# DEEPDIP-project/IncompressibleNavierStokes.jl

Hardware: AMD Instinct MI355X
Metric: M lattice-cell updates/sec (RK4 step incl. Poisson), 3D TGV fp64 (higher is better)
Workload: dtype f64; 1 GPU; TaylorGreenVortex3D 256^3 periodic fp64, RK44 + spectral Poisson, dt=0.001, Re=1e3; decomposition=single GPU, loop=timesteps_ (K steps, one native call)

## Files before the change

include/ins_hip.h:

```cpp
#ifndef INS_HIP_H
#define INS_HIP_H

#include <stdint.h>

#ifdef __cplusplus
extern "C" {
#endif

#define INS_OK 0
#define INS_ERR_INVALID (-1)
#define INS_ERR_HIP (-2)
#define INS_ERR_FFT (-3)
#define INS_ERR_UNSUPPORTED (-4)
#define INS_ERR_NOCONV (-5)
#define INS_ERR_COMM (-6)

#define INS_BC_PERIODIC 0
#define INS_BC_DIRICHLET 1
#define INS_BC_SYMMETRIC 2
#define INS_BC_PRESSURE 3
#define INS_BC_HALO 4

typedef struct ins_grid ins_grid_t;
typedef struct ins_poisson ins_poisson_t;
// ... 77 lines not shown

int ins_rk_create(const ins_grid_t* grid, ins_poisson_t* ps, int nstage, const double* A, const double* c, ins_rk_t** out);
int ins_rk_destroy(ins_rk_t* rk);
int ins_rk_step_f64(ins_rk_t* rk, double visc, double* u, double t, double dt, const double* const* planes, void* stream);
int ins_rk_step_bc_f64(ins_rk_t* rk, double visc, double* u, double t, double dt, const double* const* planes_by_time, void* stream);
int ins_rk_steps_f64(ins_rk_t* rk, double visc, double* u, double t, double dt, int nsteps, void* stream);
int ins_combine_f64(const ins_grid_t* grid, const double* base, double* out, int nterms, const double* coefs,
                    const double* const* ks, void* stream);
int ins_rk_profile_enable(ins_rk_t* rk, int enable);
int ins_rk_profile_read(ins_rk_t* rk, double* momentum_ms, int64_t* momentum_launches);
int ins_rk_set_bodyforce(ins_rk_t* rk, const double* force);

int ins_dbg_stage_rhs_used(const ins_rk_t* rk, int64_t* launches);
int ins_dbg_stage_rhs(ins_rk_t* rk, double visc, const double* u_in, const double* pI, const double* ustart, const double* kterm, double coef_k,
                      double self_in, double coef_self, double* ustar, double* rhs, int32_t* used, void* stream);
int ins_rk_pressure(const ins_rk_t* rk, double** p);
int ins_rk_stage_force(const ins_rk_t* rk, int i, double** ku);

int ins_vorticity_f64(const ins_grid_t* grid, const double* u, double* w, void* stream);
int ins_interpolate_u_p_f64(const ins_grid_t* grid, const double* u, double* up, void* stream);
int ins_interpolate_w_p_f64(const ins_grid_t* grid, const double* w, double* wp, void* stream);
int ins_dfield_f64(const ins_grid_t* grid, const double* p, double* G, double* d, double eps, void* stream);
int ins_qfield_f64(const ins_grid_t* grid, const double* u, double* Q, void* stream);
int ins_dissipation_from_strain_f64(const ins_grid_t* grid, double visc, const double* u, double* eps_out, void* stream);
int ins_eig2field_f64(const ins_grid_t* grid, const double* u, double* lam, void* stream);
int ins_apply_bc_temp_f64(const ins_grid_t* grid, const int32_t* bc, const double* val, const double* const* planes, double* temp, void* stream);
int ins_convection_diffusion_temp_f64(const ins_grid_t* grid, double a4, const double* u, const double* temp, double* c, void* stream);
int ins_dissipation_f64(const ins_grid_t* grid, double visc, double coef, const double* u, double* diff, double* diss, void* stream);
int ins_gravity_f64(const ins_grid_t* grid, int gdir, double a2, const double* temp, double* F, void* stream);
int ins_smagtensor_f64(const ins_grid_t* grid, double theta, const double* u, double* sigma, void* stream);
// ... 132 lines not shown
```

incompressiblenavierstokes.jl_amd/_lib.py:

```python
import ctypes as C
import os

_HERE = os.path.dirname(os.path.abspath(__file__))
LIB_PATH = os.environ.get("INS_HIP_LIB") or os.path.join(_HERE, "libinship.so")

INS_BC_PERIODIC, INS_BC_DIRICHLET, INS_BC_SYMMETRIC, INS_BC_PRESSURE, INS_BC_HALO = range(5)

c_double_p = C.POINTER(C.c_double)
vp = C.c_void_p


class GridDesc(C.Structure):

    _fields_ = [
        ("D", C.c_int32),
        ("N", C.c_int32 * 3),
        ("dx", c_double_p * 3),
        ("dxu", c_double_p * 3),
        ("A1", (c_double_p * 3) * 3),
        ("A2", (c_double_p * 3) * 3),
        ("iu_lo", (C.c_int32 * 3) * 3),
        ("iu_hi", (C.c_int32 * 3) * 3),
        ("ip_lo", C.c_int32 * 3),
        ("ip_hi", C.c_int32 * 3),
# ... 83 lines not shown
    "ins_filter_face_f64": (C.c_int, [vp, vp, C.c_int, vp, vp, vp]),
    "ins_filter_volume_f64": (C.c_int, [vp, vp, C.c_int, vp, vp, vp]),
    "ins_reconstruct_f64": (C.c_int, [vp, vp, C.c_int, vp, vp, vp]),
    "ins_filter_face_pullback_f64": (C.c_int, [vp, vp, C.c_int, vp, vp, vp]),
    "ins_filter_volume_pullback_f64": (C.c_int, [vp, vp, C.c_int, vp, vp, vp]),
    "ins_rk_create": (C.c_int, [vp, vp, C.c_int, c_double_p, c_double_p, C.POINTER(vp)]),
    "ins_rk_destroy": (C.c_int, [vp]),
    "ins_rk_step_f64": (C.c_int, [vp, C.c_double, vp, C.c_double, C.c_double, C.POINTER(vp), vp]),
    "ins_rk_step_bc_f64": (C.c_int, [vp, C.c_double, vp, C.c_double, C.c_double, C.POINTER(vp), vp]),
    "ins_rk_steps_f64": (C.c_int, [vp, C.c_double, vp, C.c_double, C.c_double, C.c_int, vp]),
    "ins_combine_f64": (C.c_int, [vp, vp, vp, C.c_int, c_double_p, C.POINTER(vp), vp]),
    "ins_rk_profile_enable": (C.c_int, [vp, C.c_int]),
    "ins_rk_profile_read": (C.c_int, [vp, c_double_p, C.POINTER(C.c_int64)]),
    "ins_rk_set_bodyforce": (C.c_int, [vp, vp]),
    "ins_dbg_stage_rhs_used": (C.c_int, [vp, C.POINTER(C.c_int64)]),
    "ins_dbg_stage_rhs": (C.c_int, [vp, C.c_double, vp, vp, vp, vp, C.c_double, C.c_double, C.c_double, vp, vp, C.POINTER(C.c_int32), vp]),
    "ins_rk_pressure": (C.c_int, [vp, C.POINTER(vp)]),
    "ins_rk_stage_force": (C.c_int, [vp, C.c_int, C.POINTER(vp)]),
    "ins_rk_set_temperature": (C.c_int, [vp, vp]),
    "ins_rk_set_closure": (C.c_int, [vp, C.c_int32, C.c_double]),
    "ins_rk_step_ext_f64": (C.c_int, [vp, C.c_double, vp, vp, C.c_double, C.c_double, vp]),
    "ins_stage_momentum_f64": (C.c_int, [vp, C.c_double, vp, vp, vp, vp, C.c_int, c_double_p, C.POINTER(vp), C.c_double, vp]),
    "ins_stage_momentum_corr_f64": (C.c_int, [vp, C.c_double, vp, vp, vp, vp, vp, C.c_int, c_double_p, C.POINTER(vp), C.c_double, vp]),
    "ins_stage_momentum_corr_part_f64": (C.c_int, [vp, C.c_double, vp, vp, vp, vp, vp, C.c_int, c_double_p, C.POINTER(vp), C.c_double, C.c_double, C.c_double, vp, C.c_int, vp]),
    "ins_slab_divergence_f64": (C.c_int, [vp, vp, vp, vp]),
    "ins_slab_applypressure_f64": (C.c_int, [vp, vp, vp, vp, vp]),
    "ins_slab_fft_create": (C.c_int, [C.POINTER(C.c_int32), c_double_p, C.c_int, C.c_int, C.POINTER(vp)]),
    "ins_slab_fft_destroy": (C.c_int, [vp]),
    "ins_slab_fft_sizes": (C.c_int, [vp, C.POINTER(C.c_int64), C.POINTER(C.c_int64)]),
    "ins_slab_fft_forward_xy": (C.c_int, [vp, vp, vp, vp, vp]),
# ... 136 lines not shown
```

incompressiblenavierstokes.jl_amd/csrc/ins_flux64.hip:

```cpp
#include <algorithm>
#include <cstdlib>
#include <cstring>

#include "ins_internal.h"
#include "ins_wave64.h"
#include "ins_flux_common.h"

namespace {

template <typename T, int R>
struct Plane {
  T v[3][R + 2];
  T h[3];
  T raw[3][R];
  T vm2;
  T rawv0;
};

template <typename T, int R>
struct TExt {
  T t[R + 2];
  T th;
  T vm1;
};

template <typename T, int R, int XW, bool FUSE, int CORR, bool SKEL = false, int NW = 4, bool EXTRA = false, bool RHS = false>
__global__ __launch_bounds__(64 * NW, NW == 16 ? 4 : 2) void k_flux64(FluxArgs a) {
  static_assert(!RHS || (FUSE && CORR <= 1 && !SKEL && !EXTRA), "right-hand side in the stage kernel: fused epilogue, periodic box, no extra terms");
  constexpr unsigned EB = (unsigned)sizeof(T);
  const T* const a_u = static_cast<const T*>(a.u);
  const T* const a_pI = static_cast<const T*>(a.pI);
  T* const a_F = static_cast<T*>(a.F);
  static_assert(R + 2 + (CORR ? 1 : 0) <= 8, "packed halo rows live in 8-lane groups");
  int txi, tyi, tzi;
  {
    const int nty_local = (a.nty + 7) >> 3;
    int seq = (int)(blockIdx.x >> 3);
    if (seq >= a.ntx * nty_local * a.ntz) return;
    txi = seq % a.ntx;
    seq /= a.ntx;
    tyi = (int)(blockIdx.x & 7) * nty_local + seq % nty_local;
    tzi = seq / nty_local;
    if (tyi >= a.nty) return;
// ... 69 lines not shown
    const rsrc_t rt = plane_rsrc(static_cast<const T*>((const void*)a.te.temp) + po, ubytes);
#pragma unroll
    for (int rr = 0; rr < R + 2; ++rr) E.t[rr] = ldb<T>(rt, ucol, urow[rr]);
    E.th = ldb<T>(rt, uhoff, 0);
    E.vm1 = ldb<T>(plane_rsrc(a_u + po + a.sc, ubytes), ucol, urowm1);
  };
  constexpr int NPR = R + 3 + (RHS ? 1 : 0);
  auto load_p = [&](T (&P)[NPR], T& PH, int kk) {
    const rsrc_t rs = plane_rsrc(a_pI + (long long)(CORR == 2 ? min(kk, N2) : wrapi(kk - 1, n2)) * n0 * n1, qbytes);
#pragma unroll
    for (int rr = 0; rr < R + 3; ++rr) P[rr] = ldb<T>(rs, qcol, qrow[rr]);
    PH = ldb<T>(rs, qhoff, 0);
    if constexpr (RHS) P[R + 3] = ldb<T>(rs, qcol, qrowm2);
  };
  auto correct = [&](Plane<T, R>& P, const T (&Pc)[NPR], T PHc, const T (&Pn)[NPR], T PHn) {
    if (a.epi.self_in != 0.0) {
#pragma unroll
      for (int c = 0; c < 3; ++c)
#pragma unroll
        for (int rr = 0; rr < R; ++rr) P.raw[c][rr] = P.v[c][rr + 1];
      if constexpr (RHS) P.rawv0 = P.v[1][0];
    }
    if constexpr (RHS) P.vm2 -= (Pc[0] - Pc[R + 3]) * Y.gs;
#pragma unroll
    for (int rr = 0; rr < R + 2; ++rr) {
      const T pc = Pc[rr];
      P.v[0][rr] -= (next_h(pc, rdlane(PHc, 16 + rr)) - pc) * X.gs;
      P.v[1][rr] -= (Pc[rr + 1] - pc) * Y.gs;
      P.v[2][rr] -= (Pn[rr] - pc) * Z.gs;
    }
    P.h[0] -= (dpp_old<0x108>(PHc, PHc) - PHc) * X.gs;
// ... 257 lines not shown
              if (xout && j < n1) {
                const long long pk = (long long)k * sz;
                if (a.te.ktemp_out) stb(plane_rsrc(static_cast<T*>((void*)a.te.ktemp_out) + pk, ubytes), ocol, orow[rr - 1], kt);
                stb(plane_rsrc(static_cast<T*>((void*)a.te.temp_out) + pk, ubytes), ocol, orow[rr - 1], tacc[rr - 1] + (T)a.te.c_self * kt);
              }
              wv_o = wv;
              wwprev[rr - 1] = ww;
              Tz[rr - 1] = Tc;
            }
          }
          Pz[0][rr - 1] = Uc;
          Pz[1][rr - 1] = Vc;
          Pz[2][rr - 1] = Wc;
        }
        emit(rr, k, fu, fv, fw, FUSE ? sacc[0][rr - 1] : (T)0, FUSE ? sacc[1][rr - 1] : (T)0, FUSE ? sacc[2][rr - 1] : (T)0, st);
        if constexpr (RHS) {
          const T su = sacc[0][rr - 1] + (T)a.epi.coef_self * fu, sv = sacc[1][rr - 1] + (T)a.epi.coef_self * fv, sw = sacc[2][rr - 1] + (T)a.epi.coef_self * fw;
          us_u[rr - 1] = su;
          dvs[rr - 1] = sv - vs_o;
          dws[rr - 1] = sw - wsprev[rr - 1];
          vs_o = sv;
          wsprev[rr - 1] = sw;
          if (lane == 63) rhs_lds[((k & 1) * NW + wave) * R + rr - 1] = su;
        }
      } else if constexpr (RHS) {
        const T fyv_m = flux(cvm2, Vc, cvm2, Vc, Y.vs);
        const T fxv = flux(Vc, Vn, Uc, C.v[0][rr + 1], X.vo);
        const T lxv = flux(rdlane(ch1, rr), Vc, rdlane(ch0, rr), rdlane(ch0, rr + 1), X.vo);
        T fv = (fxv - prev_h(fxv, lxv)) * X.ro;
        fv += (fyv - fyv_m) * Y.rs;
// ... 165 lines not shown
        INS_LAUNCH_CHECK();
        return INS_OK;
      }
      if (corr_mode == 1) {
        hipLaunchKernelGGL((k_flux64<T, R, XW, true, 1, false, NW, true>), dim3(nb), block, (size_t)g_lds, s, a);
        INS_LAUNCH_CHECK();
        return INS_OK;
      }
    }
    ins_set_error("stage kernel with an extra force term: fp64, fused epilogue, 2 rows, 4 wavefronts, no slab correction");
    return INS_ERR_UNSUPPORTED;
  }
  if (corr_mode == 0)
    hipLaunchKernelGGL((k_flux64<T, R, XW, FUSE, 0, false, NW>), dim3(nb), block, (size_t)g_lds, s, a);
  else if constexpr (FUSE && R <= 5) {
    if (corr_mode == 1)
      hipLaunchKernelGGL((k_flux64<T, R, XW, true, 1, false, NW>), dim3(nb), block, (size_t)g_lds, s, a);
    else
      hipLaunchKernelGGL((k_flux64<T, R, XW, true, 2, false, NW>), dim3(nb), block, (size_t)g_lds, s, a);
  } else {
    ins_set_error("in-kernel pressure correction needs the fused epilogue and <= 5 rows per thread");
    return INS_ERR_UNSUPPORTED;
  }
  INS_LAUNCH_CHECK();
  return INS_OK;
}

constexpr int ZB = 4;
template <typename T, int R, int XW, bool FUSE, int NW = 4>
int launch(const ins_grid* G, FluxArgs& a, int corr_mode, int part, hipStream_t s) {
  const GridDev& g = G->g;
// ... 6 lines not shown
  if (part != 0 && nzl <= 2 * ZB) {
    if (part == 1) return INS_OK;
    part = 0;
  }
  if (part == 1) {
    a.k_lo = 1 + ZB;
    a.k_hi = nzl + 1 - ZB;
  } else if (part == 2) {
    a.zc = ZB;
    a.kB = nzl + 1 - ZB;
  }
  a.ntz = part == 2 ? 2 : cdiv(a.k_hi - a.k_lo, a.zc);
  return launch_range<T, R, XW, FUSE, NW>(G, a, corr_mode, s);
}

template <int R, int XW, int NW, int CORR>
int launch_rhs(const ins_grid* G, FluxArgs& a, hipStream_t s) {
  const GridDev& g = G->g;
  a.ntx = 1;
  a.nty = cdiv(g.N[1] - 2, (NW / XW) * R);
  a.k_lo = 1;
  a.k_hi = g.N[2] - 1;
  a.kB = 0;
  a.ntz = cdiv(a.k_hi - a.k_lo, a.zc);
  const unsigned nb = (unsigned)(8LL * ((a.nty + 7) / 8) * a.ntz);
  hipLaunchKernelGGL((k_flux64<double, R, XW, true, CORR, false, NW, false, true>), dim3(nb), dim3(64, NW, 1), 0, s, a);
  INS_LAUNCH_CHECK();
  return INS_OK;
}

}

extern "C" void ins_tune_flux64(int disable, int rows, int rows_corr, int zchunk, int xw, int skel, int burst_unused, int lds) {
  if (disable >= 0) ins_set_option("INS_DISABLE_FLUX64", disable);
  if (rows >= 0) ins_set_option("INS_FLUX64_ROWS", rows);
  if (rows_corr >= 0) ins_set_option("INS_FLUX64_ROWS_CORR", rows_corr);
  if (zchunk >= 0) ins_set_option("INS_FLUX64_ZC", zchunk);
  if (xw >= 0) ins_set_option("INS_FLUX64_XW", xw);
  if (skel >= 0) ins_set_option("INS_FLUX64_SKEL", skel);
  (void)burst_unused;
  if (lds >= 0) ins_set_option("INS_FLUX64_LDS", lds);
// ... 54 lines not shown
    if (!zco) zc = n2 >= 128 ? 32 : (n2 >= 64 ? 16 : (n2 >= 32 ? 8 : 4));
  }
  return TileShape{xw, rows, nw, zc};
}

bool ins_flux128_supported(const ins_grid* G, const RkEpi* epi, int corr_mode, bool f32);
bool ins_flux64_stage_rhs_supported(const ins_grid* G, int corr_mode) {
  if (ins_opt(OPT_INS_DISABLE_STAGE_RHS) || corr_mode < 0 || corr_mode > 1 || !ins_flux64_supported(G) || g_skel || g_lds) return false;
  if (ins_flux128_supported(G, nullptr, corr_mode, false)) return false;
  const TileShape t = tile_shape(G, corr_mode, false, false, true);
  if (64 * t.xw != G->g.N[0] - 2) return false;
  if (corr_mode == 0) return t.rows == 4 && t.xw == 2 && t.nw == 4;
  return t.rows == 2 && ((t.xw == 3 && t.nw == 6) || ((t.xw == 2 || t.xw == 4) && (t.nw == 4 || t.nw == 8)));
}

template <typename T>
static int flux64_dispatch(const ins_grid* G, double visc, const T* u, T* F, const RkEpi* epi, const T* pI, int corr_mode, hipStream_t s, int part) {
  const GridDev& g = G->g;
  FluxArgs a;
  memset(&a, 0, sizeof(a));
  a.u = u;
  a.pI = pI;
  a.F = F;
  a.sc = g.sc;
  a.N0 = g.N[0];
  a.N1 = g.N[1];
  a.N2 = g.N[2];
  a.X = make_dir(G, 0, visc);
  a.Y = make_dir(G, 1, visc);
  a.Z = make_dir(G, 2, visc);
// ... 22 lines not shown
          if (xw == 4) return launch<T, RR, 4, FUSE, 16>(G, a, corr_mode, part, s);   \
          if (xw == 2) return launch<T, RR, 2, FUSE, 16>(G, a, corr_mode, part, s);   \
          return launch<T, RR, 1, FUSE, 16>(G, a, corr_mode, part, s);                \
        }                                                                             \
      }                                                                               \
      if (nw >= 8) {                                                                  \
        if (xw == 4) return launch<T, RR, 4, FUSE, 8>(G, a, corr_mode, part, s);      \
        if (xw == 2) return launch<T, RR, 2, FUSE, 8>(G, a, corr_mode, part, s);      \
        return launch<T, RR, 1, FUSE, 8>(G, a, corr_mode, part, s);                   \
      }                                                                               \
      if (xw == 4) return launch<T, RR, 4, FUSE>(G, a, corr_mode, part, s);           \
      if (xw == 2) return launch<T, RR, 2, FUSE>(G, a, corr_mode, part, s);           \
      return launch<T, RR, 1, FUSE>(G, a, corr_mode, part, s);                        \
    }                                                                                 \
  }
  if (want_rhs) {
    if (ins_stage_out_aliases_input(*epi, u)) {
      ins_set_error("stage kernel asked for the Poisson right-hand side while u* overwrites one of its inputs");
      return INS_ERR_INVALID;
    }
    if constexpr (!F32) {
      if (part == 0 && ins_flux64_stage_rhs_supported(G, corr_mode)) {
        a.rdiv[0] = 1.0 / G->desc.dx[0][1];
        a.rdiv[1] = 1.0 / G->desc.dx[1][1];
        a.rdiv[2] = 1.0 / G->desc.dx[2][1];
        a.om = G->desc.dx[0][1] * G->desc.dx[1][1] * G->desc.dx[2][1];
        if (corr_mode == 0) return launch_rhs<4, 2, 4, 0>(G, a, s);
        if (xw == 3) return launch_rhs<2, 3, 6, 1>(G, a, s);
        if (xw == 4) return nw == 8 ? launch_rhs<2, 4, 8, 1>(G, a, s) : launch_rhs<2, 4, 4, 1>(G, a, s);
        return nw == 8 ? launch_rhs<2, 2, 8, 1>(G, a, s) : launch_rhs<2, 2, 4, 1>(G, a, s);
      }
    }
    ins_set_error("stage kernel asked for the Poisson right-hand side on a box or tile shape it does not write it for");
    return INS_ERR_UNSUPPORTED;
  }
  if (epi) {
    INS_F64_CASE(2, true)
    INS_F64_CASE(3, true)
    INS_F64_CASE(4, true)
    INS_F64_CASE(5, true)
    INS_F64_CASE(6, true)
  } else {
// ... 1 lines not shown
    INS_F64_CASE(3, false)
    INS_F64_CASE(4, false)
    INS_F64_CASE(5, false)
    INS_F64_CASE(6, false)
  }
#undef INS_F64_CASE
  return INS_ERR_INVALID;
}

bool ins_flux128_supported(const ins_grid* G, const RkEpi* epi, int corr_mode, bool f32);
int ins_k_flux128(const ins_grid* G, double visc, const double* u, double* F, const RkEpi* epi, const double* pI, int corr_mode, hipStream_t s, int part);
int ins_k_flux128_f32(const ins_grid* G, double visc, const float* u, float* F, const RkEpi* epi, const float* pI, int corr_mode, hipStream_t s, int part);

int ins_k_flux64(const ins_grid* G, double visc, const double* u, double* F, const RkEpi* epi, const double* pI, int corr_mode, hipStream_t s,
                 int part) {
  if (ins_flux128_supported(G, epi, corr_mode, false)) return ins_k_flux128(G, visc, u, F, epi, pI, corr_mode, s, part);
  return flux64_dispatch<double>(G, visc, u, F, epi, pI, corr_mode, s, part);
}
int ins_k_flux64_f32(const ins_grid* G, double visc, const float* u, float* F, const RkEpi* epi, const float* pI, int corr_mode, hipStream_t s,
                     int part) {
  if (ins_flux128_supported(G, epi, corr_mode, true) && !ins_opt(OPT_INS_F32_ONE_COLUMN)) return ins_k_flux128_f32(G, visc, u, F, epi, pI, corr_mode, s, part);
  return flux64_dispatch<float>(G, visc, u, F, epi, pI, corr_mode, s, part);
}
```

incompressiblenavierstokes.jl_amd/csrc/ins_internal.h:

```cpp
#pragma once

#include <hip/hip_runtime.h>
#include <hipfft/hipfft.h>

#include <cstdint>
#include <cstdio>
#include <cstring>
#include <string>
#include <vector>

#include "ins_hip.h"

#define INS_EPS 2.220446049250313e-16
#define INS_MAX_STAGES 16

void ins_set_error(const char* fmt, ...);

#define INS_HIP_TRY(expr)                                                                   \
  do {                                                                                      \
    hipError_t _e = (expr);                                                                 \
    if (_e != hipSuccess) {                                                                 \
      ins_set_error("%s:%d: %s -> %s", __FILE__, __LINE__, #expr, hipGetErrorString(_e));   \
      return INS_ERR_HIP;                                                                   \
    }                                                                                       \
// ... 69 lines not shown
  X(INS_FLUX64_LDS)              \
  X(INS_FLUX64_SKEL)             \
  X(INS_FLUX64_NW)               \
  X(INS_FLUX64_NT)               \
  X(INS_FLUX64_NOBAR)            \
  X(INS_FLUX64_MINTILES)         \
  X(INS_FLUX64_XW_CORR)          \
  X(INS_UNIFORM_BITWISE)         \
  X(INS_PHAT_DENSE)              \
  X(INS_DISABLE_FDM_FUSED)       \
  X(INS_DISABLE_FDM_FOLD)        \
  X(INS_DISABLE_FDM_UNFOLD4)     \
  X(INS_DISABLE_FDM_FOLDFUSE)    \
  X(INS_DISABLE_INKERNEL_CORR)   \
  X(INS_DISABLE_STAGE_RHS)       \
  X(INS_RK_KEEP_K)               \
  X(INS_DISABLE_EXT_FUSED)       \
  X(INS_EXT_TEMP_SPLIT)          \
  X(INS_DISABLE_FUSED_RK)        \
  X(INS_DISABLE_STEP_CHAIN)      \
  X(INS_DISABLE_STEP_GRAPH)      \
  X(INS_DISABLE_LINE3)           \
  X(INS_DISABLE_XYFUSED)         \
  X(INS_DISABLE_CORR2D)          \
  X(INS_SPECTRUM_ROCFFT)         \
  X(INS_X_SKEL)                  \
  X(INS_LINE3_TK)                \
  X(INS_LINE3_WGS)               \
  X(INS_STEP_GRAPH)              \
  X(INS_ZSOLVE_SKEL)             \
// ... 123 lines not shown

struct ins_rk_ext;
void ins_rk_ext_free(ins_rk_ext* e);
struct ins_rk {
  const ins_grid* grid;
  ins_poisson* ps;
  int nstage;
  std::vector<double> A, c;
  double* ustart = nullptr;
  std::vector<double*> ku;
  double* p = nullptr;
  double* ub[2] = {nullptr, nullptr};
  std::vector<double*> vb;
  const double* force = nullptr;
  ins_rk_ext* ext = nullptr;
  long long stage_rhs_launches = 0;
  bool profiling = false;
  std::vector<hipEvent_t> prof_events;
  void* step_graph = nullptr;
};

struct Rec {
  double vs, vo, a0, b0, a1, b1, a2, b2, rs, ro, pad[6];
};

struct RkEpi {
  int n;
  int write_k;
  double coef[INS_MAX_STAGES + 1];
  const double* k[INS_MAX_STAGES + 1];
  double coef_self;
  double self_in;
  double c0m1;
  const double* ustart;
  double* ustar;
  double* ustart_out;
  double* rhs_out;
  const double* extra;
  const double* gtemp;
  double ga2;
  int gdir;
  double* wout;
  const struct TempEpi* tstage;
};

static inline bool ins_stage_out_aliases_input(const RkEpi& epi, const void* in) {
  bool a = (const void*)epi.ustar == in || epi.ustar == epi.ustart;
  for (int q = 0; q < epi.n; ++q) a = a || epi.ustar == epi.k[q];
  return a;
}

struct TempEpi {
  const double* temp;
  const double* tempstart;
  double* temp_out;
  double* ktemp_out;
  int n;
  double coef[INS_MAX_STAGES];
  const double* k[INS_MAX_STAGES];
  double c_self, a4, dcoef;
};


// ... 13 lines not shown
int ins_k_project_periodic_solve_only_2d(const ins_grid* G, ins_poisson* ps, const double* u, hipStream_t s);
int ins_k_momentum_rk_fused_generic(const ins_grid* G, double visc, const double* u_in, double* k_out, const RkEpi& epi, hipStream_t s);
int ins_k_momentum_rk_fused_corr(const ins_grid* G, double visc, const double* ustar_prev, const double* pI, double* k_out, const RkEpi& epi,
                                 hipStream_t s);
int ins_k_momentum_rk_fused_corr_slab(const ins_grid* G, double visc, const double* ustar_prev, const double* p_ext, double* k_out,
                                      const RkEpi& epi, hipStream_t s, int part = 0);
bool ins_corr3_supported(const ins_grid* G);
int ins_k_momentum_rk_fused_corr3(const ins_grid* G, double visc, const double* ustar_prev, const double* p_padded, double* k_out, const RkEpi& epi,
                                  hipStream_t s);
bool ins_k_project_fdm_fused(const ins_poisson* ps);
int ins_k_project_fdm_solve_only(const ins_grid* G, ins_poisson* ps, const double* u, double* p, hipStream_t s);
int ins_k_project_periodic_fused_2d(const ins_grid* G, ins_poisson* ps, double* u, double* p, bool keep_p, hipStream_t s);
bool ins_poisson_own2d(const ins_poisson* ps);
int ins_k_project_periodic_solve_only(const ins_grid* G, ins_poisson* ps, const double* u, hipStream_t s, const double* rhs = nullptr);
bool ins_flux64_stage_rhs_supported(const ins_grid* G, int corr_mode);
double* ins_poisson_stage_rhs(ins_poisson* ps);
int ins_k_poisson_solve(ins_poisson* ps, double* p, hipStream_t s);
bool ins_fast3d_supported(const ins_grid* G);

static inline bool ins_rk_fused3d(const ins_rk* rk) {
  const ins_grid* G = rk->grid;
  bool ok = !ins_opt(OPT_INS_DISABLE_FUSED_RK) && G->g.D == 3 && G->all_periodic && G->all_dof && rk->ps->kind == POISSON_SPECTRAL && ins_fast3d_supported(G);
  for (int a = 0; ok && a < 3; ++a) ok = rk->ps->np[a] >= 2;
  return ok;
}
static inline bool ins_rk_fused2d(const ins_rk* rk) {
  return !ins_opt(OPT_INS_DISABLE_FUSED_RK) && rk->grid->g.D == 2 && ins_poisson_own2d(rk->ps) && ins_flux2d_supported(rk->grid);
}
static inline bool ins_rk_inkernel3d(const ins_rk* rk) {
  const ins_grid* G = rk->grid;
// ... 66 lines not shown
```

incompressiblenavierstokes.jl_amd/csrc/ins_rk.hip:

```cpp
#include <cstdlib>

#include "ins_internal.h"
#include "ins_rk_terms.h"

int ins_k_momentum_generic(const ins_grid* G, double visc, const double* u, double* F, hipStream_t s);
int ins_k_momentum_fast3d(const ins_grid* G, double visc, const double* u, double* F, hipStream_t s);
int ins_k_momentum_fast3d_opts(const ins_grid* G, double visc, const double* u, double* F, bool zero_shell, hipStream_t s);
bool ins_flux64_supported(const ins_grid* G);

int ins_k_momentum_rk_fused(const ins_grid* G, double visc, const double* u_in, double* k_out, const RkEpi& epi, hipStream_t s);
int ins_k_project_periodic_fused(const ins_grid* G, ins_poisson* ps, double* u, double* p, bool keep_p, hipStream_t s, double* uout = nullptr,
                                 const double* rhs = nullptr);

int ins_k_momentum(const ins_grid* G, double visc, const double* u, double* F, hipStream_t s) {
  if (ins_fast3d_supported(G)) return ins_k_momentum_fast3d(G, visc, u, F, s);
  return ins_k_momentum_generic(G, visc, u, F, s);
}

namespace {

struct Combine {
  int n;
  double coef[INS_MAX_STAGES + 1];
  const double* k[INS_MAX_STAGES + 1];
// ... 121 lines not shown
  return INS_OK;
}

extern "C" int ins_rk_pressure(const ins_rk_t* rk, double** p) {
  INS_REQUIRE(rk && p, "null argument");
  *p = rk->p;
  return INS_OK;
}

extern "C" int ins_dbg_stage_rhs_used(const ins_rk_t* rk, int64_t* launches) {
  INS_REQUIRE(rk && launches, "null argument");
  *launches = (int64_t)rk->stage_rhs_launches;
  return INS_OK;
}

extern "C" int ins_dbg_stage_rhs(ins_rk_t* rk, double visc, const double* u_in, const double* pI, const double* ustart, const double* kterm, double coef_k,
                                 double self_in, double coef_self, double* ustar, double* rhs, int32_t* used, void* stream) {
  INS_REQUIRE(rk && u_in && ustar && rhs && used, "null argument");
  const ins_grid* G = rk->grid;
  hipStream_t s = as_stream(stream);
  RkEpi epi;
  memset(&epi, 0, sizeof(epi));
  epi.ustart = ustart;
  epi.ustar = ustar;
  epi.coef_self = coef_self;
  if (ustart) {
    epi.self_in = self_in;
    epi.c0m1 = -self_in;
  }
  if (kterm) {
// ... 90 lines not shown
  if (!raw_in && (rc = ins_k_apply_bc_u(G, u, 0, nullptr, s))) return rc;
  const bool inkernel = ins_rk_inkernel3d(rk);
  const bool vbasis = inkernel && !ins_opt(OPT_INS_RK_KEEP_K) && ins_rk_vbasis_possible(rk->A.data(), ns);
  if (vbasis && (int)rk->vb.size() < ns - 1) {
    rk->vb.resize(ns - 1, nullptr);
    for (int m = 0; m < ns - 1; ++m)
      if (!rk->vb[m]) {
        if (m < 2 && rk->ub[m]) {
          rk->vb[m] = rk->ub[m];
          continue;
        }
        INS_HIP_TRY(hipMalloc(&rk->vb[m], vbytes));
        INS_HIP_TRY(hipMemsetAsync(rk->vb[m], 0, vbytes, s));
      }
  }
  const double* in = u;
  for (int i = 0; i < ns; ++i) {
    double* out = (i == ns - 1 && ns > 1) ? u : (vbasis ? rk->vb[i] : rk->ub[i & 1]);
    RkEpi epi = ins_rk_stage_terms(rk->A.data(), ns, i, dt, vbasis ? rk->vb.data() : rk->ku.data(), rk->force, vbasis ? RK_V_BASIS : RK_K_BASIS,
                                   vbasis && ins_flux64_supported(G), RK_FORCE_DIAG_FIRST);
    epi.ustart = (i == 0) ? nullptr : (raw_in ? rk->ustart : u);
    epi.ustar = out;
    if (i == 0 && raw_in) epi.ustart_out = rk->ustart;
    const bool corr = inkernel && (i > 0 || raw_in);
    if (!ins_stage_out_aliases_input(epi, in) && ins_flux64_stage_rhs_supported(G, corr ? 1 : 0) && (epi.rhs_out = ins_poisson_stage_rhs(rk->ps)))
      ++rk->stage_rhs_launches;
    rc = timed_stage(rk, s, [&] {
      return corr ? ins_k_momentum_rk_fused_corr(G, visc, in, rk->ps->pI, rk->ku[i], epi, s) : ins_k_momentum_rk_fused(G, visc, in, rk->ku[i], epi, s);
    });
    if (rc) return rc;
    rc = (inkernel && (i < ns - 1 || raw_out)) ? ins_k_project_periodic_solve_only(G, rk->ps, out, s, epi.rhs_out)
                                               : ins_k_project_periodic_fused(G, rk->ps, out, rk->p, i == ns - 1, s, nullptr, epi.rhs_out);
    if (rc) return rc;
    in = out;
  }
  if (ns == 1) INS_HIP_TRY(hipMemcpyAsync(u, rk->ub[0], vbytes, hipMemcpyDeviceToDevice, s));
  return INS_OK;
}

static int rk_step_fused_periodic_2d(ins_rk* rk, double visc, double* u, double dt, hipStream_t s, int chain = 0) {
// ... 231 lines not shown
```

incompressiblenavierstokes.jl_amd/csrc/ins_rk_terms.h:

```cpp
#pragma once

#include "ins_internal.h"

static inline bool ins_rk_vbasis_possible(const double* A, int ns) {
  for (int m = 0; m < ns; ++m)
    if (A[m * ns + m] == 0.0) return false;
  return true;
}

static inline bool ins_rk_needed_later(const double* A, int ns, int i) {
  for (int i2 = i + 1; i2 < ns; ++i2)
    if (A[i2 * ns + i] != 0.0) return true;
  return false;
}

enum RkBasis { RK_K_BASIS, RK_V_BASIS };
enum RkForceOrder { RK_FORCE_DIAG_FIRST, RK_FORCE_INDEX_ORDER };

template <typename P>
static inline RkEpi ins_rk_stage_terms(const double* A, int ns, int i, double dt, P* const* prev, const P* force, RkBasis basis, bool input_in_regs,
                                       RkForceOrder order) {
  RkEpi epi;
  memset(&epi, 0, sizeof(epi));
  const double* row = A + i * ns;
  auto term = [&](double coef, const P* k) {
    epi.coef[epi.n] = coef;
    epi.k[epi.n] = reinterpret_cast<const double*>(k);
    ++epi.n;
  };
  if (basis == RK_V_BASIS) {
    double beta[INS_MAX_STAGES];
    for (int m = i - 1; m >= 0; --m) {
      double v = row[m];
      for (int j = m + 1; j < i; ++j) v -= beta[j] * A[j * ns + m];
      beta[m] = v / A[m * ns + m];
    }
    for (int m = 0; m < i; ++m) {
      if (beta[m] == 0.0) continue;
      epi.c0m1 -= beta[m];
      if (m == i - 1 && input_in_regs)
        epi.self_in = beta[m];
      else
        term(beta[m], prev[m]);
    }
  } else {
    for (int j = 0; j < i; ++j) {
      const double coef = dt * row[j];
      if (coef != 0.0) term(coef, prev[j]);
    }
    epi.write_k = ins_rk_needed_later(A, ns, i);
  }
  if (force) {
    double cf = order == RK_FORCE_DIAG_FIRST ? dt * row[i] : 0.0;
    if (basis == RK_K_BASIS)
      for (int j = 0; j < i; ++j) cf += dt * row[j];
    if (order == RK_FORCE_INDEX_ORDER) cf += dt * row[i];
    term(cf, force);
  }
  epi.coef_self = dt * row[i];
  return epi;
}

template <typename S, typename P>
static inline int ins_rk_sum_terms(const double* A, int ns, int i, S dt, P* const* prev, const P* force, S* coef, const P** k) {
  int n = 0;
  S cf = 0;
  for (int j = 0; j <= i; ++j) {
    const S c = dt * (S)A[i * ns + j];
    cf += c;
    if (c == 0) continue;
    coef[n] = c;
    k[n] = prev[j];
    ++n;
  }
  if (force) {
    coef[n] = cf;
    k[n] = force;
// ... 5 lines not shown
```

Before: 6879 M cell-updates/s.

## Carry RK stage combination forward from stage j to the final stage

In the v-basis RK path, the stage kernel at stage ns-3 now also writes a precombined vector (start state, its input, and its u* terms) into a spare buffer. The last stage then reads only that carried buffer plus its own input, so it no longer loads several earlier stage vectors. This aims to cut global memory reads in the bandwidth-bound final stage. The cost is an extra store in the earlier stage, one more kernel template instantiation, and the carry only applies to specific tile shapes and RK tableaux.

```diff
diff --git a/include/ins_hip.h b/include/ins_hip.h
--- a/include/ins_hip.h
+++ b/include/ins_hip.h
@@ -115,6 +115,7 @@
 int ins_dbg_stage_rhs_used(const ins_rk_t* rk, int64_t* launches);
 int ins_dbg_stage_rhs(ins_rk_t* rk, double visc, const double* u_in, const double* pI, const double* ustart, const double* kterm, double coef_k,
                       double self_in, double coef_self, double* ustar, double* rhs, int32_t* used, void* stream);
+int ins_dbg_stage_carry_used(const ins_rk_t* rk, int64_t* launches);
 int ins_rk_pressure(const ins_rk_t* rk, double** p);
 int ins_rk_stage_force(const ins_rk_t* rk, int i, double** ku);
 
diff --git a/incompressiblenavierstokes.jl_amd/_lib.py b/incompressiblenavierstokes.jl_amd/_lib.py
--- a/incompressiblenavierstokes.jl_amd/_lib.py
+++ b/incompressiblenavierstokes.jl_amd/_lib.py
@@ -121,6 +121,7 @@
     "ins_rk_profile_read": (C.c_int, [vp, c_double_p, C.POINTER(C.c_int64)]),
     "ins_rk_set_bodyforce": (C.c_int, [vp, vp]),
     "ins_dbg_stage_rhs_used": (C.c_int, [vp, C.POINTER(C.c_int64)]),
+    "ins_dbg_stage_carry_used": (C.c_int, [vp, C.POINTER(C.c_int64)]),
     "ins_dbg_stage_rhs": (C.c_int, [vp, C.c_double, vp, vp, vp, vp, C.c_double, C.c_double, C.c_double, vp, vp, C.POINTER(C.c_int32), vp]),
     "ins_rk_pressure": (C.c_int, [vp, C.POINTER(vp)]),
     "ins_rk_stage_force": (C.c_int, [vp, C.c_int, C.POINTER(vp)]),
diff --git a/incompressiblenavierstokes.jl_amd/csrc/ins_flux64.hip b/incompressiblenavierstokes.jl_amd/csrc/ins_flux64.hip
--- a/incompressiblenavierstokes.jl_amd/csrc/ins_flux64.hip
+++ b/incompressiblenavierstokes.jl_amd/csrc/ins_flux64.hip
@@ -24,9 +24,10 @@
   T vm1;
 };
 
-template <typename T, int R, int XW, bool FUSE, int CORR, bool SKEL = false, int NW = 4, bool EXTRA = false, bool RHS = false>
+template <typename T, int R, int XW, bool FUSE, int CORR, bool SKEL = false, int NW = 4, bool EXTRA = false, bool RHS = false, bool CARRY = false>
 __global__ __launch_bounds__(64 * NW, NW == 16 ? 4 : 2) void k_flux64(FluxArgs a) {
   static_assert(!RHS || (FUSE && CORR <= 1 && !SKEL && !EXTRA), "right-hand side in the stage kernel: fused epilogue, periodic box, no extra terms");
+  static_assert(!CARRY || (FUSE && CORR == 1 && !SKEL && !EXTRA && NW <= 8 && sizeof(T) == 8), "carried combination: the fp64 periodic correcting stage kernel");
   constexpr unsigned EB = (unsigned)sizeof(T);
   const T* const a_u = static_cast<const T*>(a.u);
   const T* const a_pI = static_cast<const T*>(a.pI);
@@ -126,7 +127,7 @@
     if constexpr (RHS) P[R + 3] = ldb<T>(rs, qcol, qrowm2);
   };
   auto correct = [&](Plane<T, R>& P, const T (&Pc)[NPR], T PHc, const T (&Pn)[NPR], T PHn) {
-    if (a.epi.self_in != 0.0) {
+    if (CARRY || a.epi.self_in != 0.0) {
 #pragma unroll
       for (int c = 0; c < 3; ++c)
 #pragma unroll
@@ -414,6 +415,14 @@
           Pz[2][rr - 1] = Wc;
         }
         emit(rr, k, fu, fv, fw, FUSE ? sacc[0][rr - 1] : (T)0, FUSE ? sacc[1][rr - 1] : (T)0, FUSE ? sacc[2][rr - 1] : (T)0, st);
+        if constexpr (CARRY) {
+          if (xout && jb0 + rr - 1 < n1 && st) {
+            const T ca0 = (T)a.epi.ca[0], ca1 = (T)a.epi.ca[1], ca2 = (T)a.epi.ca[2], cs = (T)a.epi.coef_self;
+            const T s0 = sacc[0][rr - 1], s1 = sacc[1][rr - 1], s2 = sacc[2][rr - 1];
+            st3(static_cast<T*>((void*)a.epi.carry_out) + (long long)k * sz, ocol, orow[rr - 1], ca0 * s0 + ca1 * C.raw[0][rr - 1] + ca2 * (s0 + cs * fu),
+                ca0 * s1 + ca1 * C.raw[1][rr - 1] + ca2 * (s1 + cs * fv), ca0 * s2 + ca1 * C.raw[2][rr - 1] + ca2 * (s2 + cs * fw));
+          }
+        }
         if constexpr (RHS) {
           const T su = sacc[0][rr - 1] + (T)a.epi.coef_self * fu, sv = sacc[1][rr - 1] + (T)a.epi.coef_self * fv, sw = sacc[2][rr - 1] + (T)a.epi.coef_self * fw;
           us_u[rr - 1] = su;
@@ -609,7 +618,14 @@
   if (corr_mode == 0)
     hipLaunchKernelGGL((k_flux64<T, R, XW, FUSE, 0, false, NW>), dim3(nb), block, (size_t)g_lds, s, a);
   else if constexpr (FUSE && R <= 5) {
-    if (corr_mode == 1)
+    if (corr_mode == 1 && a.epi.carry_out) {
+      if constexpr (R == 2 && NW <= 8 && sizeof(T) == 8) {
+        hipLaunchKernelGGL((k_flux64<T, R, XW, true, 1, false, NW, false, false, true>), dim3(nb), block, (size_t)g_lds, s, a);
+      } else {
+        ins_set_error("stage kernel asked to carry a combination forward on a tile shape it does not do it for");
+        return INS_ERR_UNSUPPORTED;
+      }
+    } else if (corr_mode == 1)
       hipLaunchKernelGGL((k_flux64<T, R, XW, true, 1, false, NW>), dim3(nb), block, (size_t)g_lds, s, a);
     else
       hipLaunchKernelGGL((k_flux64<T, R, XW, true, 2, false, NW>), dim3(nb), block, (size_t)g_lds, s, a);
@@ -646,7 +662,7 @@
   return launch_range<T, R, XW, FUSE, NW>(G, a, corr_mode, s);
 }
 
-template <int R, int XW, int NW, int CORR>
+template <int R, int XW, int NW, int CORR, bool CARRY = false>
 int launch_rhs(const ins_grid* G, FluxArgs& a, hipStream_t s) {
   const GridDev& g = G->g;
   a.ntx = 1;
@@ -656,7 +672,7 @@
   a.kB = 0;
   a.ntz = cdiv(a.k_hi - a.k_lo, a.zc);
   const unsigned nb = (unsigned)(8LL * ((a.nty + 7) / 8) * a.ntz);
-  hipLaunchKernelGGL((k_flux64<double, R, XW, true, CORR, false, NW, false, true>), dim3(nb), dim3(64, NW, 1), 0, s, a);
+  hipLaunchKernelGGL((k_flux64<double, R, XW, true, CORR, false, NW, false, true, CARRY>), dim3(nb), dim3(64, NW, 1), 0, s, a);
   INS_LAUNCH_CHECK();
   return INS_OK;
 }
@@ -741,6 +757,13 @@
   return t.rows == 2 && ((t.xw == 3 && t.nw == 6) || ((t.xw == 2 || t.xw == 4) && (t.nw == 4 || t.nw == 8)));
 }
 
+bool ins_flux64_stage_carry_supported(const ins_grid* G) {
+  if (ins_opt(OPT_INS_DISABLE_STAGE_CARRY) || !ins_flux64_supported(G) || g_skel) return false;
+  if (ins_flux128_supported(G, nullptr, 1, false)) return false;
+  const TileShape t = tile_shape(G, 1, false, false, false);
+  return t.rows == 2 && t.nw <= 8;
+}
+
 template <typename T>
 static int flux64_dispatch(const ins_grid* G, double visc, const T* u, T* F, const RkEpi* epi, const T* pI, int corr_mode, hipStream_t s, int part) {
   const GridDev& g = G->g;
@@ -793,6 +816,17 @@
       return launch<T, RR, 1, FUSE>(G, a, corr_mode, part, s);                        \
     }                                                                                 \
   }
+  const bool carry = epi && epi->carry_out;
+  if (carry) {
+    if (ins_stage_carry_aliases(*epi, u) || ins_stage_out_aliases_input(*epi, u)) {
+      ins_set_error("stage kernel asked to carry a combination forward into, or to store u* over, one of its inputs");
+      return INS_ERR_INVALID;
+    }
+    if (F32 || corr_mode != 1 || part != 0 || !ins_flux64_stage_carry_supported(G)) {
+      ins_set_error("stage kernel asked to carry a combination forward on a path that does not do it");
+      return INS_ERR_UNSUPPORTED;
+    }
+  }
   if (want_rhs) {
     if (ins_stage_out_aliases_input(*epi, u)) {
       ins_set_error("stage kernel asked for the Poisson right-hand side while u* overwrites one of its inputs");
@@ -805,6 +839,11 @@
         a.rdiv[2] = 1.0 / G->desc.dx[2][1];
         a.om = G->desc.dx[0][1] * G->desc.dx[1][1] * G->desc.dx[2][1];
         if (corr_mode == 0) return launch_rhs<4, 2, 4, 0>(G, a, s);
+        if (carry) {
+          if (xw == 3) return launch_rhs<2, 3, 6, 1, true>(G, a, s);
+          if (xw == 4) return nw == 8 ? launch_rhs<2, 4, 8, 1, true>(G, a, s) : launch_rhs<2, 4, 4, 1, true>(G, a, s);
+          return nw == 8 ? launch_rhs<2, 2, 8, 1, true>(G, a, s) : launch_rhs<2, 2, 4, 1, true>(G, a, s);
+        }
         if (xw == 3) return launch_rhs<2, 3, 6, 1>(G, a, s);
         if (xw == 4) return nw == 8 ? launch_rhs<2, 4, 8, 1>(G, a, s) : launch_rhs<2, 4, 4, 1>(G, a, s);
         return nw == 8 ? launch_rhs<2, 2, 8, 1>(G, a, s) : launch_rhs<2, 2, 4, 1>(G, a, s);
@@ -836,7 +875,13 @@
 
 int ins_k_flux64(const ins_grid* G, double visc, const double* u, double* F, const RkEpi* epi, const double* pI, int corr_mode, hipStream_t s,
                  int part) {
-  if (ins_flux128_supported(G, epi, corr_mode, false)) return ins_k_flux128(G, visc, u, F, epi, pI, corr_mode, s, part);
+  if (ins_flux128_supported(G, epi, corr_mode, false)) {
+    if (epi && epi->carry_out) {
+      ins_set_error("stage kernel asked to carry a combination forward on a path that does not do it");
+      return INS_ERR_UNSUPPORTED;
+    }
+    return ins_k_flux128(G, visc, u, F, epi, pI, corr_mode, s, part);
+  }
   return flux64_dispatch<double>(G, visc, u, F, epi, pI, corr_mode, s, part);
 }
 int ins_k_flux64_f32(const ins_grid* G, double visc, const float* u, float* F, const RkEpi* epi, const float* pI, int corr_mode, hipStream_t s,
diff --git a/incompressiblenavierstokes.jl_amd/csrc/ins_internal.h b/incompressiblenavierstokes.jl_amd/csrc/ins_internal.h
--- a/incompressiblenavierstokes.jl_amd/csrc/ins_internal.h
+++ b/incompressiblenavierstokes.jl_amd/csrc/ins_internal.h
@@ -107,6 +107,7 @@
   X(INS_DISABLE_FDM_FOLDFUSE)    \
   X(INS_DISABLE_INKERNEL_CORR)   \
   X(INS_DISABLE_STAGE_RHS)       \
+  X(INS_DISABLE_STAGE_CARRY)     \
   X(INS_RK_KEEP_K)               \
   X(INS_DISABLE_EXT_FUSED)       \
   X(INS_EXT_TEMP_SPLIT)          \
@@ -260,6 +261,7 @@
   std::vector<double*> vb;
   const double* force = nullptr;
   ins_rk_ext* ext = nullptr;
+  long long stage_carry_launches = 0;
   long long stage_rhs_launches = 0;
   bool profiling = false;
   std::vector<hipEvent_t> prof_events;
@@ -281,6 +283,8 @@
   const double* ustart;
   double* ustar;
   double* ustart_out;
+  double* carry_out;
+  double ca[3];
   double* rhs_out;
   const double* extra;
   const double* gtemp;
@@ -293,6 +297,11 @@
 static inline bool ins_stage_out_aliases_input(const RkEpi& epi, const void* in) {
   bool a = (const void*)epi.ustar == in || epi.ustar == epi.ustart;
   for (int q = 0; q < epi.n; ++q) a = a || epi.ustar == epi.k[q];
+  return a;
+}
+static inline bool ins_stage_carry_aliases(const RkEpi& epi, const void* in) {
+  bool a = (const void*)epi.carry_out == in || epi.carry_out == epi.ustart || epi.carry_out == epi.ustar;
+  for (int q = 0; q < epi.n; ++q) a = a || epi.carry_out == epi.k[q];
   return a;
 }
 
@@ -336,6 +345,7 @@
 bool ins_poisson_own2d(const ins_poisson* ps);
 int ins_k_project_periodic_solve_only(const ins_grid* G, ins_poisson* ps, const double* u, hipStream_t s, const double* rhs = nullptr);
 bool ins_flux64_stage_rhs_supported(const ins_grid* G, int corr_mode);
+bool ins_flux64_stage_carry_supported(const ins_grid* G);
 double* ins_poisson_stage_rhs(ins_poisson* ps);
 int ins_k_poisson_solve(ins_poisson* ps, double* p, hipStream_t s);
 bool ins_fast3d_supported(const ins_grid* G);
diff --git a/incompressiblenavierstokes.jl_amd/csrc/ins_rk.hip b/incompressiblenavierstokes.jl_amd/csrc/ins_rk.hip
--- a/incompressiblenavierstokes.jl_amd/csrc/ins_rk.hip
+++ b/incompressiblenavierstokes.jl_amd/csrc/ins_rk.hip
@@ -159,6 +159,28 @@
   return INS_OK;
 }
 
+extern "C" int ins_dbg_stage_carry_used(const ins_rk_t* rk, int64_t* launches) {
+  INS_REQUIRE(rk && launches, "null argument");
+  *launches = (int64_t)rk->stage_carry_launches;
+  return INS_OK;
+}
+
+extern "C" int ins_dbg_rk_carry_plan(int32_t ns, const double* A, double dt, int32_t with_force, int32_t* j, int32_t* i, double* a, double* self_in,
+                                     double* coef_self, double* coef_force) {
+  INS_REQUIRE(A && j && i && a && self_in && coef_self && coef_force, "null argument");
+  INS_REQUIRE(ns >= 1 && ns <= INS_MAX_STAGES, "bad argument");
+  const RkCarryPlan pl = ins_rk_carry_plan(A, ns);
+  *j = pl.j, *i = pl.i, *self_in = 0.0, *coef_self = 0.0, *coef_force = 0.0;
+  for (int q = 0; q < 3; ++q) a[q] = pl.a[q];
+  if (pl.j < 0) return INS_OK;
+  static double slot[2];
+  const RkEpi epi = ins_rk_carry_consumer_terms<double>(A, ns, pl, dt, slot, with_force ? slot + 1 : nullptr);
+  INS_REQUIRE(epi.ustart == slot && epi.c0m1 == 0.0 && epi.n == (with_force ? 1 : 0), "consumer terms");
+  *self_in = epi.self_in, *coef_self = epi.coef_self;
+  if (with_force) *coef_force = epi.coef[0];
+  return INS_OK;
+}
+
 extern "C" int ins_dbg_stage_rhs(ins_rk_t* rk, double visc, const double* u_in, const double* pI, const double* ustart, const double* kterm, double coef_k,
                                  double self_in, double coef_self, double* ustar, double* rhs, int32_t* used, void* stream) {
   INS_REQUIRE(rk && u_in && ustar && rhs && used, "null argument");
@@ -279,16 +301,33 @@
         INS_HIP_TRY(hipMemsetAsync(rk->vb[m], 0, vbytes, s));
       }
   }
+  RkCarryPlan pl = {-1, -1, {0.0, 0.0, 0.0}};
+  if (vbasis && ins_flux64_stage_carry_supported(G)) pl = ins_rk_carry_plan(rk->A.data(), ns);
+  const bool carry = pl.j >= 0;
   const double* in = u;
   for (int i = 0; i < ns; ++i) {
-    double* out = (i == ns - 1 && ns > 1) ? u : (vbasis ? rk->vb[i] : rk->ub[i & 1]);
+    double* out = (i == ns - 1 && ns > 1) ? u : (vbasis ? rk->vb[(carry && i == pl.j + 1) ? pl.j - 1 : i] : rk->ub[i & 1]);
     RkEpi epi = ins_rk_stage_terms(rk->A.data(), ns, i, dt, vbasis ? rk->vb.data() : rk->ku.data(), rk->force, vbasis ? RK_V_BASIS : RK_K_BASIS,
                                    vbasis && ins_flux64_supported(G), RK_FORCE_DIAG_FIRST);
     epi.ustart = (i == 0) ? nullptr : (raw_in ? rk->ustart : u);
     epi.ustar = out;
+    const bool in_place = ins_stage_out_aliases_input(epi, in);
+    if (carry && i == pl.j) {
+      epi.carry_out = rk->vb[pl.j + 1];
+      for (int q = 0; q < 3; ++q) epi.ca[q] = pl.a[q];
+      if (ins_stage_carry_aliases(epi, in) || in_place) {
+        ins_set_error("carried stage combination: an output of stage %d is one of its inputs", i);
+        return INS_ERR_INVALID;
+      }
+      ++rk->stage_carry_launches;
+    }
+    if (carry && i == pl.i) {
+      epi = ins_rk_carry_consumer_terms(rk->A.data(), ns, pl, dt, rk->vb[pl.j + 1], rk->force);
+      epi.ustar = out;
+    }
     if (i == 0 && raw_in) epi.ustart_out = rk->ustart;
     const bool corr = inkernel && (i > 0 || raw_in);
-    if (!ins_stage_out_aliases_input(epi, in) && ins_flux64_stage_rhs_supported(G, corr ? 1 : 0) && (epi.rhs_out = ins_poisson_stage_rhs(rk->ps)))
+    if (!in_place && ins_flux64_stage_rhs_supported(G, corr ? 1 : 0) && (epi.rhs_out = ins_poisson_stage_rhs(rk->ps)))
       ++rk->stage_rhs_launches;
     rc = timed_stage(rk, s, [&] {
       return corr ? ins_k_momentum_rk_fused_corr(G, visc, in, rk->ps->pI, rk->ku[i], epi, s) : ins_k_momentum_rk_fused(G, visc, in, rk->ku[i], epi, s);
diff --git a/incompressiblenavierstokes.jl_amd/csrc/ins_rk_terms.h b/incompressiblenavierstokes.jl_amd/csrc/ins_rk_terms.h
--- a/incompressiblenavierstokes.jl_amd/csrc/ins_rk_terms.h
+++ b/incompressiblenavierstokes.jl_amd/csrc/ins_rk_terms.h
@@ -12,6 +12,15 @@
   for (int i2 = i + 1; i2 < ns; ++i2)
     if (A[i2 * ns + i] != 0.0) return true;
   return false;
+}
+
+static inline void ins_rk_beta(const double* A, int ns, int i, double* beta) {
+  const double* row = A + i * ns;
+  for (int m = i - 1; m >= 0; --m) {
+    double v = row[m];
+    for (int j = m + 1; j < i; ++j) v -= beta[j] * A[j * ns + m];
+    beta[m] = v / A[m * ns + m];
+  }
 }
 
 enum RkBasis { RK_K_BASIS, RK_V_BASIS };
@@ -30,11 +39,7 @@
   };
   if (basis == RK_V_BASIS) {
     double beta[INS_MAX_STAGES];
-    for (int m = i - 1; m >= 0; --m) {
-      double v = row[m];
-      for (int j = m + 1; j < i; ++j) v -= beta[j] * A[j * ns + m];
-      beta[m] = v / A[m * ns + m];
-    }
+    ins_rk_beta(A, ns, i, beta);
     for (int m = 0; m < i; ++m) {
       if (beta[m] == 0.0) continue;
       epi.c0m1 -= beta[m];
@@ -61,6 +66,53 @@
   return epi;
 }
 
+struct RkCarryPlan {
+  int j, i;
+  double a[3];
+};
+static inline RkCarryPlan ins_rk_carry_plan(const double* A, int ns) {
+  RkCarryPlan pl = {-1, -1, {0.0, 0.0, 0.0}};
+  const int i = ns - 1, j = ns - 3;
+  if (j < 1 || !ins_rk_vbasis_possible(A, ns)) return pl;
+  double bi[INS_MAX_STAGES], bj[INS_MAX_STAGES], bn[INS_MAX_STAGES];
+  ins_rk_beta(A, ns, i, bi);
+  ins_rk_beta(A, ns, j, bj);
+  ins_rk_beta(A, ns, j + 1, bn);
+  for (int m = 0; m < j; ++m)
+    if (bj[m] != 0.0) return pl;
+  for (int m = 0; m < j - 1; ++m)
+    if (bi[m] != 0.0) return pl;
+  if (bi[j] == 0.0 || bn[j - 1] != 0.0) return pl;
+  double c0m1 = 0.0;
+  for (int m = 0; m < i; ++m)
+    if (bi[m] != 0.0) c0m1 -= bi[m];
+  if (1.0 + c0m1 == 0.0) return pl;
+  pl.j = j;
+  pl.i = i;
+  pl.a[0] = 1.0 + c0m1;
+  pl.a[1] = bi[j - 1];
+  pl.a[2] = bi[j];
+  return pl;
+}
+
+template <typename P>
+static inline RkEpi ins_rk_carry_consumer_terms(const double* A, int ns, const RkCarryPlan& pl, double dt, const P* S, const P* force) {
+  RkEpi epi;
+  memset(&epi, 0, sizeof(epi));
+  const int i = pl.i;
+  double beta[INS_MAX_STAGES];
+  ins_rk_beta(A, ns, i, beta);
+  epi.ustart = reinterpret_cast<const double*>(S);
+  epi.self_in = beta[i - 1];
+  if (force) {
+    epi.coef[0] = dt * A[i * ns + i] - pl.a[0] * (dt * A[pl.j * ns + pl.j]);
+    epi.k[0] = reinterpret_cast<const double*>(force);
+    epi.n = 1;
+  }
+  epi.coef_self = dt * A[i * ns + i];
+  return epi;
+}
+
 template <typename S, typename P>
 static inline int ins_rk_sum_terms(const double* A, int ns, int i, S dt, P* const* prev, const P* force, S* coef, const P** k) {
   int n = 0;
```

Measured after the change: 7007 M cell-updates/s, median of 6. 1.9% higher.
